# clementabary/music2dance

Hardware: AMD Instinct MI355X
Metric: 120-frame seq/sec, phase3 WGAN-GP step, batch 64 per GPU (higher is better)
Workload: dtype f32

## Files before the change

### music2dance_amd/csrc/gemm_engine.hip

```cpp
#include "gemm_engine.h"
#include <atomic>
#include <map>
#include <mutex>

typedef float f32x16 __attribute__((ext_vector_type(16)));

template <int BM, int BN, int NW>
struct M2dTiling {
  static constexpr int WM = BM >= 64 ? 2 : 1;
  static constexpr int WN = NW / WM;
  static constexpr int TM = BM / (32 * WM);
  static constexpr int TN = BN / (32 * WN);
  static constexpr int NTH = 64 * NW;
};

__device__ __forceinline__ void m2d_divmod(int n, int d, float inv, int& q, int& r) {
  q = (int)((float)n * inv);
  r = n - q * d;
  const int adj = (r < 0 ? -1 : 0) + (r >= d ? 1 : 0);
  q += adj;
  r -= adj * d;
}

__device__ __forceinline__ void m2d_tile_of(int tile_map, int& bx, int& by) {
  bx = blockIdx.x;
  by = blockIdx.y;
  if (tile_map == 0) return;
  const int nt = gridDim.x, mt = gridDim.y;
  const int T = nt * mt, q = T >> 3, r = T & 7;
  const int lin = by * nt + bx;
  const int xcd = lin & 7, idx = lin >> 3;
  const int id = (xcd < r ? xcd * (q + 1) : r * (q + 1) + (xcd - r) * q) + idx;
  const int GM = 8;
  const int per = GM * nt;
  const int grp = id / per, rem = id - grp * per;
  const int first = grp * GM;
  const int gsz = mt - first < GM ? mt - first : GM;
  const int nn = rem / gsz;
  by = first + rem - nn * gsz;
  bx = nn;
}

#define M2D_OOB 0x80000000u
#define M2D_BAD 0x40000000

__device__ __forceinline__ __amdgpu_buffer_rsrc_t m2d_rsrc(const float* p, unsigned nbytes) {
  return __builtin_amdgcn_make_buffer_rsrc((void*)p, (short)0, (int)nbytes, 0x00020000);
}

__device__ __forceinline__ float m2d_bload(__amdgpu_buffer_rsrc_t r, unsigned voff, int soff) {
  return __builtin_bit_cast(float, __builtin_amdgcn_raw_buffer_load_b32(r, (int)voff, soff, 0));
}

typedef __attribute__((address_space(3))) float m2d_lds_f;
__device__ __forceinline__ void m2d_bload_lds(__amdgpu_buffer_rsrc_t r, float* dst, unsigned voff, int soff) {
  __builtin_amdgcn_raw_ptr_buffer_load_lds(r, (m2d_lds_f*)dst, 4, (int)voff, soff, 0, 0);
}

__device__ __forceinline__ int m2d_hi_offset(const M2dOperand& op, int hi) {
  if (op.rdiv2 <= 0) return hi * op.r_hi_stride;
  int q, r;
  m2d_divmod(hi, op.rdiv2, op.rdiv2_inv, q, r);
  return q * op.r_hi2_stride + r * op.r_hi_stride;
}

template <bool KF, int BR, bool MASKED, int NTH = 256>
struct TileMap {
  static constexpr int NE = BR * M2D_BK / NTH;
  static constexpr int NR = KF ? NE : 1;
  static constexpr int NM = MASKED ? NE : 1;
  unsigned eoff[NR];
  int posr;
  int kb;
  unsigned lim_eff;
  bool force_one;
  float one_val;
  float v[NE];
  float mv[NM];

  __device__ __forceinline__ void prep(const M2dOperand& op, int row0, int tid) {
    lim_eff = op.lim > 0 ? (unsigned)op.lim : (unsigned)(M2D_BAD - 1);
    force_one = false;
    one_val = 1.f;
    if constexpr (KF) {
      kb = tid % M2D_BK;
      posr = 0;
#pragma unroll
      for (int i = 0; i < NE; ++i) {
        const int g = row0 + tid / M2D_BK + i * (NTH / M2D_BK);
        const bool rv = g < op.nrows;
        int hi, lo;
        m2d_divmod(rv ? g : 0, op.rdiv, op.rdiv_inv, hi, lo);
        const int off = m2d_hi_offset(op, hi) + lo * op.r_lo_stride + op.r_off + kb * op.k_lo_stride;
        eoff[i] = rv ? ((unsigned)off << 2) : M2D_OOB;
      }
    } else {
      const int kb_t = (tid / BR) * NE;
      kb = BR >= 64 ? __builtin_amdgcn_readfirstlane(kb_t) : kb_t;
      const int g = row0 + tid % BR;
      const bool rv = g < op.nrows;
      force_one = (g + 1 == op.ones_row_p1);
      int hi, lo;
      m2d_divmod(rv ? g : 0, op.rdiv, op.rdiv_inv, hi, lo);
      const int off = m2d_hi_offset(op, hi) + lo * op.r_lo_stride + op.r_off + kb * op.k_lo_stride;
      eoff[0] = (unsigned)off << 2;
      posr = rv ? (op.lim > 0 ? lo * op.r_pos_mul + op.r_pos_off + kb * op.k_pos_lo : 0) : M2D_BAD;
    }
  }

  static constexpr int DL_KSTEP = BR >= 64 ? 1 : 64 / BR;
  __device__ __forceinline__ void prep_dl(const M2dOperand& op, int row0, int tid) {
    static_assert(!KF && !MASKED && (BR == 32 || BR >= 64), "LDS-direct staging: row-fast, unmasked");
    static_assert(BR >= 64 || NTH == 256, "32-row LDS-direct staging: four waves");
    if constexpr (BR >= 64) {
      prep(op, row0, tid);
    } else {
      lim_eff = op.lim > 0 ? (unsigned)op.lim : (unsigned)(M2D_BAD - 1);
      force_one = false;
      kb = 4 * (tid >> 6) + ((tid >> 5) & 1);
      const int g = row0 + (tid & (BR - 1));
      const bool rv = g < op.nrows;
      int hi, lo;
      m2d_divmod(rv ? g : 0, op.rdiv, op.rdiv_inv, hi, lo);
      const int off = m2d_hi_offset(op, hi) + lo * op.r_lo_stride + op.r_off + kb * op.k_lo_stride;
      eoff[0] = (unsigned)off << 2;
      posr = rv ? (op.lim > 0 ? lo * op.r_pos_mul + op.r_pos_off + kb * op.k_pos_lo : 0) : M2D_BAD;
    }
  }

  __device__ __forceinline__ void fetch(__amdgpu_buffer_rsrc_t rs, __amdgpu_buffer_rsrc_t rm, int i, unsigned voff,
                                        int soff) {
    v[i] = m2d_bload(rs, voff, soff);
    if constexpr (MASKED) mv[i] = m2d_bload(rm, voff, soff);
  }

  template <bool UNIFORM>
  __device__ __forceinline__ void load(const M2dOperand& op, __amdgpu_buffer_rsrc_t rs, __amdgpu_buffer_rsrc_t rm,
                                       int hi, int lo0, int kdiv) {
    int hoff = hi * op.k_hi_stride;
    if (op.kdiv2 > 0) {
      const int q = hi / op.kdiv2;
      hoff = q * op.k_hi2_stride + (hi - q * op.kdiv2) * op.k_hi_stride;
    }
    const int S = (hoff + lo0 * op.k_lo_stride) << 2;
    if constexpr (!KF) one_val = hi >= op.ones_from_hi ? 1.f : 0.f;
    if constexpr (KF) {
      if constexpr (UNIFORM) {
#pragma unroll
        for (int i = 0; i < NE; ++i) fetch(rs, rm, i, eoff[i], S);
      } else {
        const bool tv = lo0 + kb < kdiv;
#pragma unroll
        for (int i = 0; i < NE; ++i) fetch(rs, rm, i, tv ? eoff[i] : M2D_OOB, S);
      }
    } else {
      const int P = hi * op.k_pos_hi + lo0 * op.k_pos_lo;
      const unsigned full = eoff[0] + (unsigned)S;
      const int ls4 = op.k_lo_stride << 2;
      if constexpr (UNIFORM) {
        const unsigned voff = ((unsigned)(posr + P) < lim_eff) ? full : M2D_OOB;
#pragma unroll
        for (int i = 0; i < NE; ++i) fetch(rs, rm, i, voff, i * ls4);
      } else {
#pragma unroll
        for (int i = 0; i < NE; ++i) {
          const int pp = (lo0 + kb + i < kdiv) ? P + i * op.k_pos_lo : M2D_BAD;
          fetch(rs, rm, i, ((unsigned)(posr + pp) < lim_eff) ? full + (unsigned)(i * ls4) : M2D_OOB, 0);
        }
      }
    }
  }

  template <bool UNIFORM, int LD>
  __device__ __forceinline__ void load_lds(const M2dOperand& op, __amdgpu_buffer_rsrc_t rs, int hi, int lo0, int kdiv,
                                           float* img, int tid) const {
    static_assert(!KF && !MASKED, "LDS-direct staging: row-fast, unmasked");
    constexpr int KS = DL_KSTEP;
    int hoff = hi * op.k_hi_stride;
    const int S = (hoff + lo0 * op.k_lo_stride) << 2;
    const int P = hi * op.k_pos_hi + lo0 * op.k_pos_lo;
    const unsigned full = eoff[0] + (unsigned)S;
    const int ls4 = (op.k_lo_stride * KS) << 2;
    const int kb0 = BR >= 64 ? kb : 4 * (__builtin_amdgcn_readfirstlane(tid) >> 6);
    const int row0 = BR >= 64 ? (__builtin_amdgcn_readfirstlane(tid) & (BR - 1) & ~63) : 0;
    float* dst = img + kb0 * LD + row0;
    if constexpr (UNIFORM) {
      const unsigned voff = ((unsigned)(posr + P) < lim_eff) ? full : M2D_OOB;
#pragma unroll
      for (int i = 0; i < NE; ++i) m2d_bload_lds(rs, dst + (KS * i) * LD, voff, i * ls4);
    } else {
#pragma unroll
      for (int i = 0; i < NE; ++i) {
        const int pp = (lo0 + kb + KS * i < kdiv) ? P + (KS * i) * op.k_pos_lo : M2D_BAD;
        m2d_bload_lds(rs, dst + (KS * i) * LD, ((unsigned)(posr + pp) < lim_eff) ? full + (unsigned)(i * ls4) : M2D_OOB, 0);
      }
    }
  }

  template <int LD>
  __device__ __forceinline__ void store(const M2dOperand& op, float* s, int tid) const {
#pragma unroll
    for (int i = 0; i < NE; ++i) {
      const int kl = KF ? (tid % M2D_BK) : ((tid / BR) * NE + i);
      const int rl = KF ? (tid / M2D_BK + i * (NTH / M2D_BK)) : (tid % BR);
      float x = v[i];
      if constexpr (MASKED) x *= (mv[i] > 0.f ? 1.f : op.mask_slope);
      if constexpr (!KF) x = force_one ? one_val : x;
      s[kl * LD + rl] = x;
    }
  }
};

struct ChunkCursor {
  int hi, lo0, kdiv, nhi;
  int lo_outer;
  int a_lo, a_hi, b_lo, b_hi;
  __device__ __forceinline__ void seek(int c, int cph) {
    if (lo_outer) {
      const int blk = c / nhi;
      hi = c - blk * nhi;
      lo0 = blk * M2D_BK;
    } else {
      hi = c / cph;
      lo0 = (c - hi * cph) * M2D_BK;
    }
  }
  __device__ __forceinline__ bool past() const { return lo_outer ? lo0 >= kdiv : hi >= nhi; }
  __device__ __forceinline__ bool uniform() const {
    return (!past()) & (lo0 + M2D_BK <= kdiv) & (lo0 >= a_lo) & (lo0 + M2D_BK <= a_hi) & (lo0 >= b_lo) &
           (lo0 + M2D_BK <= b_hi);
  }
  __device__ __forceinline__ int extent() const { return past() ? 0 : kdiv; }
  __device__ __forceinline__ void next() {
    if (lo_outer) {
      hi += 1;
      const bool wrap = hi >= nhi;
      hi = wrap ? 0 : hi;
      lo0 += wrap ? M2D_BK : 0;
    } else {
      lo0 += M2D_BK;
      const bool wrap = lo0 >= kdiv;
      lo0 = wrap ? 0 : lo0;
      hi += wrap ? 1 : 0;
    }
  }
};

__device__ __forceinline__ unsigned m2d_mask_off(unsigned voff, unsigned wrapb) {
  return (voff != M2D_OOB && voff >= wrapb) ? voff - wrapb : voff;
}

__device__ __forceinline__ float m2d_epilogue(const M2dOutMap& o, float v, int row, int col, int addr) {
  const int maddr = (o.mask_wrap && addr >= (int)o.mask_wrap) ? addr - (int)o.mask_wrap : addr;
  if (o.bias_mode == 1) v += o.bias[row];
  else if (o.bias_mode == 2) v += o.bias[col];
  v = m2d_act(v, o.act, o.slope);
  if (o.mask_last) {
    if (o.residual) v += o.residual[addr];
    if (o.mask) v *= (o.mask[maddr] > 0.f ? 1.f : o.mask_slope);
    return v;
  }
  if (o.mask) v *= (o.mask[maddr] > 0.f ? 1.f : o.mask_slope);
  if (o.sum_out) {
    o.sum_out[addr] = v + o.residual[addr];
    return v;
  }
  if (o.residual) v += o.residual[addr];
  return v;
}

template <int BM, int BN, bool AKF, bool BKF, bool MASKED>
__device__ __forceinline__ void m2d_chunk_mma(const TileMap<AKF, BM, MASKED>& ta, const TileMap<BKF, BN, MASKED>& tb,
                                              const M2dOperand& A, const M2dOperand& B, float* smem, int cur,
                                              int tid, int wm, int wn, int l31, int lh,
                                              f32x16 (&acc)[BM / (32 * (BM >= 64 ? 2 : 1))][BN / (32 * (4 / (BM >= 64 ? 2 : 1)))]) {
  constexpr int LDA = BM + M2D_LDPAD;
  constexpr int LDB = BN + M2D_LDPAD;
  constexpr int WM = BM >= 64 ? 2 : 1;
  constexpr int WN = 4 / WM;
  constexpr int TM = BM / (32 * WM);
  constexpr int TN = BN / (32 * WN);
  constexpr int STAGE = M2D_BK * (LDA + LDB);
  const float* as = smem + cur * STAGE + wm * (TM * 32) + l31;
  const float* bs = smem + cur * STAGE + M2D_BK * LDA + wn * (TN * 32) + l31;
  float fa[M2D_BK / 2][TM], fb[M2D_BK / 2][TN];
#pragma unroll
  for (int kk = 0; kk < M2D_BK / 2; ++kk) {
#pragma unroll
    for (int i = 0; i < TM; ++i) fa[kk][i] = as[(2 * kk + lh) * LDA + i * 32];
#pragma unroll
    for (int j = 0; j < TN; ++j) fb[kk][j] = bs[(2 * kk + lh) * LDB + j * 32];
  }
#pragma unroll
  for (int kk = 0; kk < M2D_BK / 2; ++kk)
#pragma unroll
    for (int i = 0; i < TM; ++i)
#pragma unroll
      for (int j = 0; j < TN; ++j)
        acc[i][j] = __builtin_amdgcn_mfma_f32_32x32x2f32(fa[kk][i], fb[kk][j], acc[i][j], 0, 0, 0);
  float* nxt = smem + (cur ^ 1) * STAGE;
  ta.template store<LDA>(A, nxt, tid);
  tb.template store<LDB>(B, nxt + M2D_BK * LDA, tid);
  __builtin_amdgcn_sched_group_barrier(0x100, 4, 0);
#pragma unroll
  for (int kk = 0; kk < M2D_BK / 2; ++kk) {
    __builtin_amdgcn_sched_group_barrier(0x008, TM * TN, 0);
    if (kk < M2D_BK / 2 - 2) __builtin_amdgcn_sched_group_barrier(0x100, 2, 0);
  }
}

template <int BM, int BN, int NW = 4>
__device__ __forceinline__ void m2d_acc_init(const M2dGemmParams& p, const M2dOutMap& O, int N, int split, int m0, int n0, int wm,
                                             int wn, int l31, int lh,
                                             f32x16 (&acc)[M2dTiling<BM, BN, NW>::TM][M2dTiling<BM, BN, NW>::TN]) {
  constexpr int TM = M2dTiling<BM, BN, NW>::TM;
  constexpr int TN = M2dTiling<BM, BN, NW>::TN;
  const bool with_bias = O.bias_mode != 0 && (p.splits <= 1 || (p.tickets && split == 0));
  if (!with_bias) {
#pragma unroll
    for (int i = 0; i < TM; ++i)
#pragma unroll
      for (int j = 0; j < TN; ++j)
#pragma unroll
        for (int r = 0; r < 16; ++r) acc[i][j][r] = 0.f;
    return;
  }
  if (O.bias_mode == 1) {
#pragma unroll
    for (int i = 0; i < TM; ++i)
#pragma unroll
      for (int r = 0; r < 16; ++r) {
        const int row = m0 + wm * (TM * 32) + i * 32 + (r & 3) + 8 * (r >> 2) + 4 * lh;
        const float b = row < p.M ? O.bias[row] : 0.f;
#pragma unroll
        for (int j = 0; j < TN; ++j) acc[i][j][r] = b;
      }
  } else {
#pragma unroll
    for (int j = 0; j < TN; ++j) {
      const int col = n0 + wn * (TN * 32) + j * 32 + l31;
      const float b = col < N ? O.bias[col] : 0.f;
#pragma unroll
      for (int i = 0; i < TM; ++i)
#pragma unroll
        for (int r = 0; r < 16; ++r) acc[i][j][r] = b;
    }
  }
}

__device__ __forceinline__ float4 m2d_ld4(const float* p) { return *reinterpret_cast<const float4*>(p); }
__device__ __forceinline__ void m2d_st4(float* p, float4 v) { *reinterpret_cast<float4*>(p) = v; }

typedef unsigned int m2d_u32x4 __attribute__((__vector_size__(16)));
typedef float m2d_vf32x4 __attribute__((__vector_size__(16)));
__device__ __forceinline__ void m2d_bstore1(__amdgpu_buffer_rsrc_t r, unsigned voff, float v) {
  __builtin_amdgcn_raw_buffer_store_b32(__builtin_bit_cast(unsigned, v), r, (int)voff, 0, 0);
}
__device__ __forceinline__ void m2d_bstore4(__amdgpu_buffer_rsrc_t r, unsigned voff, float4 v) {
  m2d_vf32x4 w;
  w[0] = v.x; w[1] = v.y; w[2] = v.z; w[3] = v.w;
  __builtin_amdgcn_raw_buffer_store_b128(__builtin_bit_cast(m2d_u32x4, w), r, (int)voff, 0, 0);
}
__device__ __forceinline__ float4 m2d_bload4(__amdgpu_buffer_rsrc_t r, unsigned voff) {
  const m2d_vf32x4 w = __builtin_bit_cast(m2d_vf32x4, __builtin_amdgcn_raw_buffer_load_b128(r, (int)voff, 0, 0));
  return make_float4(w[0], w[1], w[2], w[3]);
}

template <int BM, int BN, bool WIDE, int NW = 4>
__device__ __forceinline__ void m2d_tile_epilogue(const M2dGemmParams& p, const M2dOutMap& O, int N, int split, int m0,
                                                  int n0, int wm, int wn, int lane, float* wl,
                                                  f32x16 (&acc)[M2dTiling<BM, BN, NW>::TM][M2dTiling<BM, BN, NW>::TN]) {
  constexpr int WN = M2dTiling<BM, BN, NW>::WN;
  constexpr int TM = M2dTiling<BM, BN, NW>::TM;
  constexpr int TN = M2dTiling<BM, BN, NW>::TN;
  const int l31 = lane & 31, lh = lane >> 5;
  const bool slab = p.splits > 1 && !p.tickets;
  const bool stats = O.row_part != nullptr && !slab;
  const bool has_mask = O.mask != nullptr && !slab, has_res = O.residual != nullptr && !slab;
  const bool two_out = O.sum_out != nullptr && !slab;
  const int act = slab ? 0 : O.act;
  const float ms = O.mask_slope;
  const int m_stride = slab ? p.N : O.m_stride;
  const int m_div = slab ? 0 : O.m_div;
  const int c_lim = slab ? 0 : O.c_lim;
  const int redirect = slab ? 0 : O.redirect_col_p1;
  const float* out_base = slab ? p.slab + (size_t)split * p.M * p.N : O.out;
#define M2D_RS(ptr) m2d_rsrc((ptr), 0x7ffffffcu)
  constexpr int NT = (BM == 128 && WIDE) ? TN : 1;
  const int rl0 = lane >> 3, c4 = (lane & 7) * 4;
  constexpr int PER_TILE = WIDE ? 4 : 16;
  constexpr int ITEMS = NT * PER_TILE;
  constexpr int GROUP = WIDE ? ITEMS : (BM == 128 ? 8 : 16);
#pragma unroll
  for (int i = 0; i < TM; ++i) {
    const int rowb = m0 + wm * (TM * 32) + i * 32;
#pragma unroll
    for (int j0 = 0; j0 < TN; j0 += NT) {
#pragma unroll
      for (int jj = 0; jj < NT; ++jj)
#pragma unroll
        for (int r = 0; r < 16; ++r) wl[jj * 1024 + ((r & 3) + 8 * (r >> 2) + 4 * lh) * 32 + l31] = acc[i][j0 + jj][r];
      __builtin_amdgcn_fence(__ATOMIC_RELEASE, "wavefront");
      __builtin_amdgcn_wave_barrier();
      __builtin_amdgcn_sched_barrier(0);
      int caddr_t[NT], pos_t[NT];
      bool cok_t[NT], red_t[NT];
#pragma unroll
      for (int jj = 0; jj < NT; ++jj) {
        const int col = n0 + wn * (TN * 32) + (j0 + jj) * 32 + (WIDE ? c4 : l31);
        const bool cv = col < N;
        if (slab) {
          caddr_t[jj] = col;
          pos_t[jj] = 0;
        } else {
          int chi, clo;
          m2d_divmod(cv ? col : 0, O.cdiv, O.cdiv_inv, chi, clo);
          caddr_t[jj] = chi * O.c_hi_stride + clo * (WIDE ? 1 : O.c_lo_stride) + O.c_off;
          pos_t[jj] = clo * O.c_pos_mul + O.c_pos_off;
        }
        red_t[jj] = !WIDE && cv && (col + 1 == redirect);
        bool cok = cv;
        if (!WIDE && c_lim > 0 && m_div <= 0) cok = cok && ((unsigned)pos_t[jj] < (unsigned)c_lim);
        cok_t[jj] = cok;
      }
      {
        bool fast = !has_res && m_div <= 0;
        if constexpr (!WIDE) fast = fast && (!stats || (!has_mask && c_lim <= 0 && (p.stats_narrow_fast != 0))) && __ballot(red_t[0]) == 0ull;
        if (fast) {
          if constexpr (!WIDE) {
            if (stats) {
#pragma unroll
              for (int jj = 0; jj < NT; ++jj) {
                const int colb = n0 + wn * (TN * 32) + (j0 + jj) * 32 + c4;
#pragma unroll
                for (int it = 0; it < 4; ++it) {
                  const int rl = rl0 + 8 * it;
                  float4 x = m2d_ld4(wl + jj * 1024 + rl * 32 + c4);
                  x.x = colb + 0 < N ? m2d_act_sel(x.x, act, O.slope) : 0.f;
                  x.y = colb + 1 < N ? m2d_act_sel(x.y, act, O.slope) : 0.f;
                  x.z = colb + 2 < N ? m2d_act_sel(x.z, act, O.slope) : 0.f;
                  x.w = colb + 3 < N ? m2d_act_sel(x.w, act, O.slope) : 0.f;
                  float a1 = (x.x + x.y) + (x.z + x.w);
                  float a2 = (x.x * x.x + x.y * x.y) + (x.z * x.z + x.w * x.w);
#pragma unroll
                  for (int off = 4; off > 0; off >>= 1) {
                    a1 += __shfl_xor(a1, off, 64);
                    a2 += __shfl_xor(a2, off, 64);
                  }
                  if ((lane & 7) == 0 && rowb + rl < p.M) {
                    float* dst = O.row_part + ((size_t)(((n0 / BN) * WN + wn) * TN + j0 + jj) * p.M + rowb + rl) * 2;
                    dst[0] = a1;
                    dst[1] = a2;
                  }
                }
              }
            }
          }
          const __amdgpu_buffer_rsrc_t rso = m2d_rsrc(out_base, 0x7ffffffcu);
#pragma unroll
          for (int jj = 0; jj < NT; ++jj) {
            constexpr int NI = PER_TILE;
            constexpr int RS = WIDE ? 8 : 2;
            const int r0 = WIDE ? rl0 : lh;
            const unsigned step = (unsigned)(RS * m_stride) << 2;
            const unsigned v0 = cok_t[jj] ? (unsigned)((rowb + r0) * m_stride + caddr_t[jj]) << 2 : M2D_OOB;
            const int nrow = p.M - rowb - r0;
            unsigned keep = 0xffffffffu;
            if (has_mask) {
              const __amdgpu_buffer_rsrc_t rsm = m2d_rsrc(O.mask, 0x7ffffffcu);
              const unsigned wrapb = O.mask_wrap ? O.mask_wrap * 4u : 0xffffffffu;
              keep = 0u;
              if constexpr (WIDE) {
                float4 mraw[NI];
#pragma unroll
                for (int it = 0; it < NI; ++it)
                  mraw[it] = m2d_bload4(rsm, m2d_mask_off((RS * it < nrow && v0 != M2D_OOB) ? v0 + (unsigned)it * step : M2D_OOB, wrapb));
#pragma unroll
                for (int it = 0; it < NI; ++it)
                  keep |= ((mraw[it].x > 0.f ? 1u : 0u) | (mraw[it].y > 0.f ? 2u : 0u) | (mraw[it].z > 0.f ? 4u : 0u) | (mraw[it].w > 0.f ? 8u : 0u)) << (4 * it);
              } else {
                float mraw[NI];
#pragma unroll
                for (int it = 0; it < NI; ++it)
                  mraw[it] = m2d_bload(rsm, m2d_mask_off((RS * it < nrow && v0 != M2D_OOB) ? v0 + (unsigned)it * step : M2D_OOB, wrapb), 0);
#pragma unroll
                for (int it = 0; it < NI; ++it) keep |= (mraw[it] > 0.f ? 1u : 0u) << it;
              }
            }
            const float* img = wl + jj * 1024 + r0 * 32 + (WIDE ? c4 : l31);
#pragma unroll
            for (int it = 0; it < NI; ++it) {
              const bool ok = RS * it < nrow && v0 != M2D_OOB;
              const unsigned voff = ok ? v0 + (unsigned)it * step : M2D_OOB;
              if constexpr (WIDE) {
                float4 x = m2d_ld4(img + it * (RS * 32));
                const unsigned kb = keep >> (4 * it);
                x.x = m2d_act(x.x, act, O.slope) * ((kb & 1u) ? 1.f : ms);
                x.y = m2d_act(x.y, act, O.slope) * ((kb & 2u) ? 1.f : ms);
                x.z = m2d_act(x.z, act, O.slope) * ((kb & 4u) ? 1.f : ms);
                x.w = m2d_act(x.w, act, O.slope) * ((kb & 8u) ? 1.f : ms);
                m2d_bstore4(rso, voff, x);
                if (stats) {
                  float a1 = ok ? (x.x + x.y) + (x.z + x.w) : 0.f;
                  float a2 = ok ? (x.x * x.x + x.y * x.y) + (x.z * x.z + x.w * x.w) : 0.f;
#pragma unroll
                  for (int off = 4; off > 0; off >>= 1) {
                    a1 += __shfl_xor(a1, off, 64);
                    a2 += __shfl_xor(a2, off, 64);
                  }
                  if ((lane & 7) == 0 && RS * it < nrow) {
                    float* dst = O.row_part + ((size_t)(((n0 / BN) * WN + wn) * TN + j0 + jj) * p.M + rowb + r0 + RS * it) * 2;
                    dst[0] = a1;
                    dst[1] = a2;
                  }
                }
              } else {
                float x = img[it * (RS * 32)];
                x = m2d_act_sel(x, act, O.slope) * (((keep >> it) & 1u) ? 1.f : ms);
                m2d_bstore1(rso, voff, x);
              }
            }
          }
          __builtin_amdgcn_wave_barrier();
          continue;
        }
      }
      auto locate = [&](int q, int& jj, int& rl, int& row, unsigned& voff) {
        jj = NT > 1 ? q / PER_TILE : 0;
        const int it = q - jj * PER_TILE;
        rl = WIDE ? rl0 + 8 * it : 2 * it + lh;
        row = rowb + rl;
        const int caddr = NT > 1 && jj ? caddr_t[NT - 1] : caddr_t[0];
        bool ok = row < p.M && (NT > 1 && jj ? cok_t[NT - 1] : cok_t[0]) && !(NT > 1 && jj ? red_t[NT - 1] : red_t[0]);
        int addr;
        if (!WIDE && m_div > 0) {
          int mhi, mlo;
          m2d_divmod(row, m_div, 1.f / (float)m_div, mhi, mlo);
          const int pos = NT > 1 && jj ? pos_t[NT - 1] : pos_t[0];
          if (c_lim > 0) ok = ok && ((unsigned)(pos + mlo * O.m_pos_mul) < (unsigned)c_lim);
          addr = mhi * m_stride + mlo * O.m_lo_stride + caddr;
        } else {
          addr = row * m_stride + caddr;
        }
        voff = ok ? (unsigned)addr << 2 : M2D_OOB;
      };
#pragma unroll 1
      for (int q0 = 0; q0 < ITEMS; q0 += GROUP) {
        unsigned keep = 0xffffffffu;
        if (has_mask) {
          keep = 0u;
          const unsigned wrapb = O.mask_wrap ? O.mask_wrap * 4u : 0xffffffffu;
          if constexpr (WIDE) {
            float4 mraw[GROUP];
#pragma unroll
            for (int q = 0; q < GROUP; ++q) {
              int jj, rl, row;
              unsigned voff;
              locate(q0 + q, jj, rl, row, voff);
              mraw[q] = m2d_bload4(M2D_RS(O.mask), m2d_mask_off(voff, wrapb));
            }
#pragma unroll
            for (int q = 0; q < GROUP; ++q)
              keep |= ((mraw[q].x > 0.f ? 1u : 0u) | (mraw[q].y > 0.f ? 2u : 0u) | (mraw[q].z > 0.f ? 4u : 0u) | (mraw[q].w > 0.f ? 8u : 0u)) << (4 * q);
          } else {
            float mraw[GROUP];
#pragma unroll
            for (int q = 0; q < GROUP; ++q) {
              int jj, rl, row;
              unsigned voff;
              locate(q0 + q, jj, rl, row, voff);
              mraw[q] = m2d_bload(M2D_RS(O.mask), m2d_mask_off(voff, wrapb), 0);
            }
#pragma unroll
            for (int q = 0; q < GROUP; ++q) keep |= (mraw[q] > 0.f ? 1u : 0u) << q;
          }
        }
#pragma unroll 2
        for (int qq = 0; qq < GROUP; ++qq) {
          int jj, rl, row;
          unsigned voff;
          locate(q0 + qq, jj, rl, row, voff);
          const bool ok = voff != M2D_OOB;
          float a1 = 0.f, a2 = 0.f;
          if constexpr (WIDE) {
            float4 x = m2d_ld4(wl + jj * 1024 + rl * 32 + c4);
            x.x = m2d_act(x.x, act, O.slope); x.y = m2d_act(x.y, act, O.slope);
            x.z = m2d_act(x.z, act, O.slope); x.w = m2d_act(x.w, act, O.slope);
            if (has_res && O.mask_last) {
              const float4 r4 = m2d_bload4(M2D_RS(O.residual), voff);
              x.x += r4.x; x.y += r4.y; x.z += r4.z; x.w += r4.w;
            }
            const unsigned kb = keep >> (4 * qq);
            x.x *= (kb & 1u) ? 1.f : ms; x.y *= (kb & 2u) ? 1.f : ms; x.z *= (kb & 4u) ? 1.f : ms; x.w *= (kb & 8u) ? 1.f : ms;
            if (has_res && !O.mask_last) {
              const float4 r4 = m2d_bload4(M2D_RS(O.residual), voff);
              const float4 sum = make_float4(x.x + r4.x, x.y + r4.y, x.z + r4.z, x.w + r4.w);
              if (two_out) m2d_bstore4(M2D_RS(O.sum_out), voff, sum);
              else x = sum;
            }
            m2d_bstore4(M2D_RS(out_base), voff, x);
            if (stats) {
              a1 = ok ? (x.x + x.y) + (x.z + x.w) : 0.f;
              a2 = ok ? (x.x * x.x + x.y * x.y) + (x.z * x.z + x.w * x.w) : 0.f;
#pragma unroll
              for (int off = 4; off > 0; off >>= 1) {
                a1 += __shfl_xor(a1, off, 64);
                a2 += __shfl_xor(a2, off, 64);
              }
              if ((lane & 7) == 0 && row < p.M) {
                float* dst = O.row_part + ((size_t)(((n0 / BN) * WN + wn) * TN + j0 + jj) * p.M + row) * 2;
                dst[0] = a1;
                dst[1] = a2;
              }
            }
// ... 373 lines not shown
    const int nq = top >= 0 ? (top / s - qmin + 1) : 0;
    if (nq <= 0) return;
    N = p.ph_batch * nq;
    if ((int)(bx * BN) >= N) return;
    nhi = taps;
    A.r_off += r * (p.ph_a_step ? p.ph_a_step : p.ph_cout);
    B.nrows = N;
    B.rdiv = nq;
    B.rdiv_inv = 1.f / (float)nq;
    B.r_off = qmin;
    B.r_pos_off = qmin;
    O.cdiv = nq;
    O.cdiv_inv = B.rdiv_inv;
    O.c_off = s * qmin + r - p.ph_pad;
    O.c_pos_off = O.c_off;
  }
  const int m0 = by * BM;
  const int n0 = bx * BN;
  TileMap<false, BM, false, NTH> ta;
  TileMap<false, BN, false, NTH> tb;
  ta.prep_dl(A, m0, tid);
  tb.prep_dl(B, n0, tid);
  const __amdgpu_buffer_rsrc_t ra = m2d_rsrc(A.base, A.nbytes);
  const __amdgpu_buffer_rsrc_t rb = m2d_rsrc(B.base, B.nbytes);

  f32x16 acc[TM][TN];
  if constexpr (EPI == 2) {
#pragma unroll
    for (int i = 0; i < TM; ++i)
#pragma unroll
      for (int j = 0; j < TN; ++j)
#pragma unroll
        for (int r = 0; r < 16; ++r) acc[i][j][r] = 0.f;
  } else {
    m2d_acc_init<BM, BN, NW>(p, O, N, split, m0, n0, wm, wn, l31, lh, acc);
  }

  const int cph = (p.kdiv + M2D_BK - 1) / M2D_BK;
  const int nchunks = nhi * cph;
  const int cps = (nchunks + p.splits - 1) / p.splits;
  const int c0 = split * cps;
  const int c1 = (c0 + cps < nchunks) ? (c0 + cps) : nchunks;

  if (c0 < c1) {
    ChunkCursor cc;
    cc.kdiv = p.kdiv;
    cc.nhi = nhi;
    cc.lo_outer = p.lo_outer;
    cc.seek(c0, cph);
    cc.a_lo = A.k_safe_lo; cc.a_hi = A.k_safe_hi;
    cc.b_lo = B.k_safe_lo; cc.b_hi = B.k_safe_hi;
    ta.template load_lds<false, BM>(A, ra, cc.hi, cc.lo0, cc.extent(), smem, tid);
    tb.template load_lds<false, BN>(B, rb, cc.hi, cc.lo0, cc.extent(), smem + M2D_BK * BM, tid);
    cc.next();
    asm volatile("s_waitcnt vmcnt(0)" ::: "memory");
    __syncthreads();
    M2D_STAMP_AT(1);
    for (int c = c0; c < c1; ++c) {
      const int cur = (c - c0) & 1;
      float* nxt = smem + (cur ^ 1) * STAGE;
      if (cc.uniform()) {
        ta.template load_lds<true, BM>(A, ra, cc.hi, cc.lo0, cc.kdiv, nxt, tid);
        tb.template load_lds<true, BN>(B, rb, cc.hi, cc.lo0, cc.kdiv, nxt + M2D_BK * BM, tid);
      } else {
        ta.template load_lds<false, BM>(A, ra, cc.hi, cc.lo0, cc.extent(), nxt, tid);
        tb.template load_lds<false, BN>(B, rb, cc.hi, cc.lo0, cc.extent(), nxt + M2D_BK * BM, tid);
      }
      m2d_chunk_mma_dl<BM, BN, NW>(smem + cur * STAGE, wm, wn, l31, lh, acc);
      cc.next();
      asm volatile("s_waitcnt vmcnt(0)" ::: "memory");
      __syncthreads();
    }
  }
  M2D_STAMP_AT(2);
  if (p.tickets && !m2d_splitk_fixup<BM, BN, NW>(p, split, tid, reinterpret_cast<volatile int*>(smem), acc)) return;
  if constexpr (EPI == 2) m2d_tile_epilogue_quad<BM, BN, NW>(p, O, N, m0, n0, wm, wn, l31, lh, acc);
  else m2d_tile_epilogue<BM, BN, EPI == 1, NW>(p, O, N, split, m0, n0, wm, wn, lane, smem + wave * ((BM == 128 && NW == 4) ? 2048 : 1024), acc);
#ifdef M2D_STAMP
  asm volatile("s_waitcnt vmcnt(0)" ::: "memory");
#endif
  M2D_STAMP_AT(3);
}

template <int RB>
__device__ __forceinline__ void m2d_chunk_mma_tall(const float* stage, int wn, int l31, int lh, f32x16 (&acc)[4]) {
  const float* as = stage + l31;
  const float* bs = stage + M2D_BK * 128 + wn * 32 + l31;
  float fa[M2D_BK / 2][RB], fb[M2D_BK / 2];
#pragma unroll
  for (int kk = 0; kk < M2D_BK / 2; ++kk) {
#pragma unroll
    for (int i = 0; i < RB; ++i) fa[kk][i] = as[(2 * kk + lh) * 128 + i * 32];
    fb[kk] = bs[(2 * kk + lh) * 128];
  }
#pragma unroll
  for (int kk = 0; kk < M2D_BK / 2; ++kk)
#pragma unroll
    for (int i = 0; i < RB; ++i) acc[i] = __builtin_amdgcn_mfma_f32_32x32x2f32(fa[kk][i], fb[kk], acc[i], 0, 0, 0);
  __builtin_amdgcn_sched_group_barrier(0x100, RB + 1, 0);
#pragma unroll
  for (int kk = 0; kk < M2D_BK / 2; ++kk) {
    __builtin_amdgcn_sched_group_barrier(0x008, RB, 0);
    if (kk < M2D_BK / 2 - 2) __builtin_amdgcn_sched_group_barrier(0x100, RB > 1 ? 3 : 2, 0);
  }
}

__global__ void __launch_bounds__(256, 2) m2d_gemm_dl_tall_kernel(const M2dGemmParams p) {
  constexpr int BM = 128, BN = 128;
  constexpr int STAGE = M2D_BK * (BM + BN);
  __shared__ float smem[2 * STAGE];
  const int tid = threadIdx.x;
  const int lane = tid & 63;
  const int wn = tid >> 6;
  const int l31 = lane & 31;
  const int lh = lane >> 5;
  M2D_STAMP_AT(0);
  const M2dOperand& A = p.A;
  const M2dOperand& B = p.B;
  const M2dOutMap& O = p.O;
  const int N = p.N;
  int bx, by;
  m2d_tile_of(p.tile_map, bx, by);
  const int m0 = by * BM;
  const int n0 = bx * BN;
  TileMap<false, BM, false, 256> ta;
  TileMap<false, BN, false, 256> tb;
  ta.prep_dl(A, m0, tid);
  tb.prep_dl(B, n0, tid);
  const __amdgpu_buffer_rsrc_t ra = m2d_rsrc(A.base, A.nbytes);
  const __amdgpu_buffer_rsrc_t rb = m2d_rsrc(B.base, B.nbytes);
  f32x16 acc[4];
#pragma unroll
  for (int i = 0; i < 4; ++i)
#pragma unroll
    for (int r = 0; r < 16; ++r) acc[i][r] = 0.f;

  const int nhi = p.nhi;
  const int cph = (p.kdiv + M2D_BK - 1) / M2D_BK;
  ChunkCursor cc;
  cc.kdiv = p.kdiv;
  cc.nhi = nhi;
  cc.lo_outer = 1;
  cc.seek(0, cph);
  cc.a_lo = A.k_safe_lo; cc.a_hi = A.k_safe_hi;
  cc.b_lo = B.k_safe_lo; cc.b_hi = B.k_safe_hi;
  ta.template load_lds<false, BM>(A, ra, cc.hi, cc.lo0, cc.extent(), smem, tid);
  tb.template load_lds<false, BN>(B, rb, cc.hi, cc.lo0, cc.extent(), smem + M2D_BK * BM, tid);
  cc.next();
  asm volatile("s_waitcnt vmcnt(0)" ::: "memory");
  __syncthreads();
  M2D_STAMP_AT(1);
  int cur = 0;
  auto stage_next = [&]() {
    float* nxt = smem + (cur ^ 1) * STAGE;
    if (cc.uniform()) {
      ta.template load_lds<true, BM>(A, ra, cc.hi, cc.lo0, cc.kdiv, nxt, tid);
      tb.template load_lds<true, BN>(B, rb, cc.hi, cc.lo0, cc.kdiv, nxt + M2D_BK * BM, tid);
    } else {
      ta.template load_lds<false, BM>(A, ra, cc.hi, cc.lo0, cc.extent(), nxt, tid);
      tb.template load_lds<false, BN>(B, rb, cc.hi, cc.lo0, cc.extent(), nxt + M2D_BK * BM, tid);
    }
  };
  auto step_done = [&]() {
    cc.next();
    asm volatile("s_waitcnt vmcnt(0)" ::: "memory");
    __syncthreads();
// ... 462 lines not shown
      const double lat = (double)m2d_ceil_div64(per_cu, conc) * step;
      double cost = 8.0 + cps * (thr > lat ? thr : lat);
      if (sp > 1) cost += 6.0 + slab_mul * (double)sp * (double)M * (double)N * 8.0 / 4.0e6;
      if (rm) cost = rounds_cost(*rm, b, tiles * sp, cps, sp, M, N);
      if (rm && kind == M2D_PLAN_BWD_WEIGHT && bms[b] < 128 && M >= 128) cost *= 2.0;
      all[na].bm = bms[b];
      all[na].splits = (int)sp;
      all[na].cost = cost;
      ++na;
    }
  }
  for (int i = 0; i < na; ++i)
    for (int j = i + 1; j < na; ++j)
      if (all[j].cost < all[i].cost) {
        PlanCand t = all[i];
        all[i] = all[j];
        all[j] = t;
      }
  int n = 0;
  for (int i = 0; i < na && n < M2D_MAX_CAND; ++i)
    if (all[i].cost <= 1.5 * all[0].cost + 6.0) out[n++] = all[i];
  return n;
}

#ifdef M2D_TUNING
static int g_last_plan[9];
extern "C" int m2d_debug_last_plan(int* out) {
  memcpy(out, g_last_plan, sizeof(g_last_plan));
  return M2D_OK;
}
#endif

M2dGemmPlan m2d_gemm_plan(int M, int N, int nchunks, int phases, bool allow_split, double small_tile_penalty, int kind) {
  PlanCand c[M2D_MAX_CAND];
  const int n = plan_candidates(M, N, nchunks, phases, allow_split, small_tile_penalty, c, kind);
  M2dGemmPlan pl;
  pl.bm = n ? c[0].bm : 128;
  pl.splits = n ? c[0].splits : 1;
  pl.ws_bytes = 0;
  for (int i = 0; i < n; ++i) {
    const size_t b = m2d_slab_bytes(M, N, c[i].bm, c[i].splits);
    if (b > pl.ws_bytes) pl.ws_bytes = b;
  }
#ifdef M2D_TUNING
  if (const char* e = getenv("M2D_PLAN")) {
    int bm = 0, sp = 0;
    if (sscanf(e, "%d,%d", &bm, &sp) == 2) {
      if (bm == 32 || bm == 64 || bm == 128) pl.bm = bm;
      if (sp >= 1 && allow_split && phases <= 1 && sp <= nchunks) pl.splits = sp;
      if (sp == 1) pl.splits = 1;
      const size_t b = m2d_slab_bytes(M, N, pl.bm, pl.splits);
      if (b > pl.ws_bytes) pl.ws_bytes = b;
    }
  }
#endif
  return pl;
}

template <int BM, bool AKF, bool BKF>
static void launch_tile(const M2dGemmParams& p, dim3 grid, hipStream_t stream) {
  const bool masked = p.A.mask || p.B.mask;
  if (masked && p.O.wide) hipLaunchKernelGGL((m2d_gemm_kernel<BM, 128, AKF, BKF, true, true>), grid, dim3(256), 0, stream, p);
  else if (masked) hipLaunchKernelGGL((m2d_gemm_kernel<BM, 128, AKF, BKF, true, false>), grid, dim3(256), 0, stream, p);
  else if (p.O.wide) hipLaunchKernelGGL((m2d_gemm_kernel<BM, 128, AKF, BKF, false, true>), grid, dim3(256), 0, stream, p);
  else hipLaunchKernelGGL((m2d_gemm_kernel<BM, 128, AKF, BKF, false, false>), grid, dim3(256), 0, stream, p);
}

static bool dl_enabled() {
  static const bool on = [] { const char* e = getenv("M2D_DL"); return !(e && e[0] == '0'); }();
  return on;
}
bool m2d_dl_enabled() { return dl_enabled(); }

static inline bool dl_eligible(const M2dGemmParams& p, bool akf, bool bkf) {
  return !akf && !bkf && !p.A.mask && !p.B.mask && !p.A.ones_row_p1 && !p.B.ones_row_p1 && p.A.rdiv2 <= 0 &&
         p.B.rdiv2 <= 0 && p.A.kdiv2 <= 0 && p.B.kdiv2 <= 0;
}

static bool dl8_enabled() {
  static const bool on = [] { const char* e = getenv("M2D_DL8"); return !(e && e[0] == '0'); }();
  return on;
}

template <int BM>
static int launch_maps(const M2dGemmParams& p, bool akf, bool bkf, dim3 grid, hipStream_t stream) {
  {
    if (dl_enabled() && dl_eligible(p, akf, bkf)) {
      if constexpr (BM == 128) {
        if (p.tall_last_rb) {
          hipLaunchKernelGGL(m2d_gemm_dl_tall_kernel, grid, dim3(256), 0, stream, p);
          return 0;
        }
        if (dl8_enabled() && (p.O.wide || (p.O.quad && p.splits <= 1))) {
          if (p.O.wide) hipLaunchKernelGGL((m2d_gemm_dl_kernel<128, 128, 1, 8>), grid, dim3(512), 0, stream, p);
          else hipLaunchKernelGGL((m2d_gemm_dl_kernel<128, 128, 2, 8>), grid, dim3(512), 0, stream, p);
          return 0;
        }
      }
      if (p.O.wide) hipLaunchKernelGGL((m2d_gemm_dl_kernel<BM, 128, 1>), grid, dim3(256), 0, stream, p);
      else if (p.O.quad && p.splits <= 1) hipLaunchKernelGGL((m2d_gemm_dl_kernel<BM, 128, 2>), grid, dim3(256), 0, stream, p);
      else hipLaunchKernelGGL((m2d_gemm_dl_kernel<BM, 128, 0>), grid, dim3(256), 0, stream, p);
      return 0;
    }
  }
  if (akf && !bkf) launch_tile<BM, true, false>(p, grid, stream);
  else if (!akf && !bkf) launch_tile<BM, false, false>(p, grid, stream);
  else if (akf && bkf) launch_tile<BM, true, true>(p, grid, stream);
  else return -1;
  return 0;
}

static std::mutex g_scratch_mu;
static std::map<hipStream_t, std::pair<unsigned*, size_t>> g_scratch;

unsigned* m2d_stream_scratch_get(hipStream_t stream, size_t* bytes) {
  std::lock_guard<std::mutex> lk(g_scratch_mu);
  auto it = g_scratch.find(stream);
  if (it == g_scratch.end()) {
    if (bytes) *bytes = 0;
    return nullptr;
  }
  if (bytes) *bytes = it->second.second;
  return it->second.first;
}

extern "C" int m2d_stream_create(void** stream) {
  if (!stream) M2D_FAIL(M2D_ERR_ARG, "m2d_stream_create: null argument");
  hipStream_t s = nullptr;
  if (hipStreamCreateWithFlags(&s, hipStreamNonBlocking) != hipSuccess) M2D_FAIL(M2D_ERR_HIP, "m2d_stream_create: hipStreamCreateWithFlags failed");
  *stream = (void*)s;
  return M2D_OK;
}

extern "C" int m2d_stream_scratch_set(void* stream, void* zeroed, size_t bytes) {
  std::lock_guard<std::mutex> lk(g_scratch_mu);
  if (!zeroed || bytes == 0) g_scratch.erase((hipStream_t)stream);
  else g_scratch[(hipStream_t)stream] = std::make_pair((unsigned*)zeroed, bytes);
  return M2D_OK;
}

struct PlanQuery {
  int nchunks, phases;
  bool allow_split;
  double small_tile_penalty;
  int kind;
  bool k4;
  void* ws;
  size_t ws_bytes;
  unsigned* tickets;
  size_t ticket_bytes;
  const char* what;
};
struct Plan {
  int bm, splits;
  unsigned* tickets;
};

static unsigned* decide_fused(const M2dGemmParams& p, const PlanQuery& q, int bm, int splits) {
  static const bool on = [] { const char* e = getenv("M2D_FUSED_SPLITK"); return !(e && e[0] == '0'); }();
  static const int max_splits = [] { const char* e = getenv("M2D_FUSE_MAX"); return e ? atoi(e) : M2D_FUSE_MAX_SPLITS; }();
  if (!on || splits <= 1 || splits > max_splits || p.bwd_data || !q.ws) return nullptr;
  const size_t need = m2d_slab_bytes(p.M, p.N, bm, splits);
  if (need > q.ws_bytes || need >= 0x7fffffffULL || ((uintptr_t)q.ws & 15u)) return nullptr;
  const size_t tiles = (size_t)m2d_ceil_div(p.M, bm) * (size_t)m2d_ceil_div(p.N, 128);
  if (!q.tickets || tiles * sizeof(unsigned) > q.ticket_bytes) return nullptr;
  return q.tickets;
}

static bool stats_split_enabled() {
  static const bool on = [] { const char* e = getenv("M2D_STATS_SPLIT"); return !(e && e[0] == '0'); }();
  return on;
}

static int select_plan(const M2dGemmParams& p, const PlanQuery& q, Plan* out) {
  const bool stats = p.O.row_part != nullptr;
  const bool allow_split = q.allow_split && !(stats && !stats_split_enabled());
// ... 189 lines not shown
```

Measured before the change: 5702.

## Add paired-row LDS-direct GEMM kernel with 16-byte A staging and interleaved rows

Adds a new 128x128 four-wave GEMM kernel for eligible problems. It stages A with 16-byte buffer-to-LDS loads and interleaves row pairs so each lane reads a float2 fragment feeding two MFMA tiles. The B loader, bias init and epilogue are adapted to the paired row mapping. The goal is fewer LDS-direct load instructions and fewer LDS reads per chunk than the 8-wave and 4-wave DL kernels, in exchange for stricter alignment and eligibility checks. It is enabled by default through an environment mask and also counts its launches.

```diff
diff --git a/music2dance_amd/csrc/gemm_engine.hip b/music2dance_amd/csrc/gemm_engine.hip
--- a/music2dance_amd/csrc/gemm_engine.hip
+++ b/music2dance_amd/csrc/gemm_engine.hip
@@ -78,6 +78,7 @@
   float v[NE];
   float mv[NM];
 
+  template <bool PAIRS = false>
   __device__ __forceinline__ void prep(const M2dOperand& op, int row0, int tid) {
     lim_eff = op.lim > 0 ? (unsigned)op.lim : (unsigned)(M2D_BAD - 1);
     force_one = false;
@@ -97,7 +98,9 @@
     } else {
       const int kb_t = (tid / BR) * NE;
       kb = BR >= 64 ? __builtin_amdgcn_readfirstlane(kb_t) : kb_t;
-      const int g = row0 + tid % BR;
+      int rl = tid % BR;
+      if constexpr (PAIRS) rl = (rl & ~63) + 32 * (tid & 1) + ((tid & 63) >> 1);
+      const int g = row0 + rl;
       const bool rv = g < op.nrows;
       force_one = (g + 1 == op.ones_row_p1);
       int hi, lo;
@@ -109,11 +112,13 @@
   }
 
   static constexpr int DL_KSTEP = BR >= 64 ? 1 : 64 / BR;
+  template <bool PAIRS = false>
   __device__ __forceinline__ void prep_dl(const M2dOperand& op, int row0, int tid) {
     static_assert(!KF && !MASKED && (BR == 32 || BR >= 64), "LDS-direct staging: row-fast, unmasked");
     static_assert(BR >= 64 || NTH == 256, "32-row LDS-direct staging: four waves");
+    static_assert(!PAIRS || BR >= 64, "paired rows: whole 64-row lines");
     if constexpr (BR >= 64) {
-      prep(op, row0, tid);
+      prep<PAIRS>(op, row0, tid);
     } else {
       lim_eff = op.lim > 0 ? (unsigned)op.lim : (unsigned)(M2D_BAD - 1);
       force_one = false;
@@ -198,6 +203,32 @@
   }
 
   template <int LD>
+  __device__ __forceinline__ void load_lds_merged(const M2dOperand& op, __amdgpu_buffer_rsrc_t rs, int hi, int lo0, int kdiv,
+                                                  bool uniform, float* img, int tid) const {
+    static_assert(!KF && !MASKED && BR >= 64, "LDS-direct staging: row-fast, unmasked, whole 64-row lines");
+    const int S = (hi * op.k_hi_stride + lo0 * op.k_lo_stride) << 2;
+    const int P = hi * op.k_pos_hi + lo0 * op.k_pos_lo;
+    const unsigned full = eoff[0] + (unsigned)S;
+    const int ls4 = op.k_lo_stride << 2;
+    float* dst = img + kb * LD + (__builtin_amdgcn_readfirstlane(tid) & (BR - 1) & ~63);
+    unsigned voff[NE];
+    if (uniform) {
+      const unsigned v = ((unsigned)(posr + P) < lim_eff) ? full : M2D_OOB;
+#pragma unroll
+      for (int i = 0; i < NE; ++i) voff[i] = v;
+    } else {
+#pragma unroll
+      for (int i = 0; i < NE; ++i) {
+        const int pp = (lo0 + kb + i < kdiv) ? P + i * op.k_pos_lo : M2D_BAD;
+        voff[i] = ((unsigned)(posr + pp) < lim_eff) ? full + (unsigned)(i * ls4) : M2D_OOB;
+      }
+    }
+    const int lsu = uniform ? ls4 : 0;
+#pragma unroll
+    for (int i = 0; i < NE; ++i) m2d_bload_lds(rs, dst + i * LD, voff[i], i * lsu);
+  }
+
+  template <int LD>
   __device__ __forceinline__ void store(const M2dOperand& op, float* s, int tid) const {
 #pragma unroll
     for (int i = 0; i < NE; ++i) {
@@ -309,7 +340,14 @@
   }
 }
 
-template <int BM, int BN, int NW = 4>
+template <bool PAIR>
+struct M2dAccRows {
+  static constexpr int STEP = PAIR ? 2 : 1;
+  static __device__ __forceinline__ int first(int w0, int i) { return PAIR ? w0 + i : w0 + 32 * i; }
+  static __device__ __forceinline__ int row(int w0, int i, int f) { return first(w0, i) + STEP * f; }
+};
+
+template <int BM, int BN, int NW = 4, bool PAIR = false>
 __device__ __forceinline__ void m2d_acc_init(const M2dGemmParams& p, const M2dOutMap& O, int N, int split, int m0, int n0, int wm,
                                              int wn, int l31, int lh,
                                              f32x16 (&acc)[M2dTiling<BM, BN, NW>::TM][M2dTiling<BM, BN, NW>::TN]) {
@@ -330,7 +368,7 @@
     for (int i = 0; i < TM; ++i)
 #pragma unroll
       for (int r = 0; r < 16; ++r) {
-        const int row = m0 + wm * (TM * 32) + i * 32 + (r & 3) + 8 * (r >> 2) + 4 * lh;
+        const int row = M2dAccRows<PAIR>::row(m0 + wm * (TM * 32), i, (r & 3) + 8 * (r >> 2) + 4 * lh);
         const float b = row < p.M ? O.bias[row] : 0.f;
 #pragma unroll
         for (int j = 0; j < TN; ++j) acc[i][j][r] = b;
@@ -366,7 +404,7 @@
   return make_float4(w[0], w[1], w[2], w[3]);
 }
 
-template <int BM, int BN, bool WIDE, int NW = 4>
+template <int BM, int BN, bool WIDE, int NW = 4, bool PAIR = false>
 __device__ __forceinline__ void m2d_tile_epilogue(const M2dGemmParams& p, const M2dOutMap& O, int N, int split, int m0,
                                                   int n0, int wm, int wn, int lane, float* wl,
                                                   f32x16 (&acc)[M2dTiling<BM, BN, NW>::TM][M2dTiling<BM, BN, NW>::TN]) {
@@ -393,7 +431,8 @@
   constexpr int GROUP = WIDE ? ITEMS : (BM == 128 ? 8 : 16);
 #pragma unroll
   for (int i = 0; i < TM; ++i) {
-    const int rowb = m0 + wm * (TM * 32) + i * 32;
+    constexpr int RM = M2dAccRows<PAIR>::STEP;
+    const int rowb = M2dAccRows<PAIR>::first(m0 + wm * (TM * 32), i);
 #pragma unroll
     for (int j0 = 0; j0 < TN; j0 += NT) {
 #pragma unroll
@@ -447,8 +486,8 @@
                     a1 += __shfl_xor(a1, off, 64);
                     a2 += __shfl_xor(a2, off, 64);
                   }
-                  if ((lane & 7) == 0 && rowb + rl < p.M) {
-                    float* dst = O.row_part + ((size_t)(((n0 / BN) * WN + wn) * TN + j0 + jj) * p.M + rowb + rl) * 2;
+                  if ((lane & 7) == 0 && rowb + RM * rl < p.M) {
+                    float* dst = O.row_part + ((size_t)(((n0 / BN) * WN + wn) * TN + j0 + jj) * p.M + rowb + RM * rl) * 2;
                     dst[0] = a1;
                     dst[1] = a2;
                   }
@@ -460,11 +499,12 @@
 #pragma unroll
           for (int jj = 0; jj < NT; ++jj) {
             constexpr int NI = PER_TILE;
-            constexpr int RS = WIDE ? 8 : 2;
+            constexpr int IS = WIDE ? 8 : 2;
+            constexpr int RS = RM * IS;
             const int r0 = WIDE ? rl0 : lh;
             const unsigned step = (unsigned)(RS * m_stride) << 2;
-            const unsigned v0 = cok_t[jj] ? (unsigned)((rowb + r0) * m_stride + caddr_t[jj]) << 2 : M2D_OOB;
-            const int nrow = p.M - rowb - r0;
+            const unsigned v0 = cok_t[jj] ? (unsigned)((rowb + RM * r0) * m_stride + caddr_t[jj]) << 2 : M2D_OOB;
+            const int nrow = p.M - rowb - RM * r0;
             unsigned keep = 0xffffffffu;
             if (has_mask) {
               const __amdgpu_buffer_rsrc_t rsm = m2d_rsrc(O.mask, 0x7ffffffcu);
@@ -493,7 +533,7 @@
               const bool ok = RS * it < nrow && v0 != M2D_OOB;
               const unsigned voff = ok ? v0 + (unsigned)it * step : M2D_OOB;
               if constexpr (WIDE) {
-                float4 x = m2d_ld4(img + it * (RS * 32));
+                float4 x = m2d_ld4(img + it * (IS * 32));
                 const unsigned kb = keep >> (4 * it);
                 x.x = m2d_act(x.x, act, O.slope) * ((kb & 1u) ? 1.f : ms);
                 x.y = m2d_act(x.y, act, O.slope) * ((kb & 2u) ? 1.f : ms);
@@ -509,13 +549,13 @@
                     a2 += __shfl_xor(a2, off, 64);
                   }
                   if ((lane & 7) == 0 && RS * it < nrow) {
-                    float* dst = O.row_part + ((size_t)(((n0 / BN) * WN + wn) * TN + j0 + jj) * p.M + rowb + r0 + RS * it) * 2;
+                    float* dst = O.row_part + ((size_t)(((n0 / BN) * WN + wn) * TN + j0 + jj) * p.M + rowb + RM * r0 + RS * it) * 2;
                     dst[0] = a1;
                     dst[1] = a2;
                   }
                 }
               } else {
-                float x = img[it * (RS * 32)];
+                float x = img[it * (IS * 32)];
                 x = m2d_act_sel(x, act, O.slope) * (((keep >> it) & 1u) ? 1.f : ms);
                 m2d_bstore1(rso, voff, x);
               }
@@ -529,7 +569,7 @@
         jj = NT > 1 ? q / PER_TILE : 0;
         const int it = q - jj * PER_TILE;
         rl = WIDE ? rl0 + 8 * it : 2 * it + lh;
-        row = rowb + rl;
+        row = rowb + RM * rl;
         const int caddr = NT > 1 && jj ? caddr_t[NT - 1] : caddr_t[0];
         bool ok = row < p.M && (NT > 1 && jj ? cok_t[NT - 1] : cok_t[0]) && !(NT > 1 && jj ? red_t[NT - 1] : red_t[0]);
         int addr;
@@ -1069,6 +1109,141 @@
   M2D_STAMP_AT(3);
 }
 
+typedef float m2d_f32x2 __attribute__((ext_vector_type(2)));
+
+__device__ __forceinline__ void m2d_chunk_mma_dlp(const float* stage, int wm, int wn, int l31, int lh, f32x16 (&acc)[2][2]) {
+  const float* as = stage + wm * 64 + 2 * l31;
+  const float* bs = stage + M2D_BK * 128 + wn * 64 + 2 * l31;
+  m2d_f32x2 fa[M2D_BK / 2], fb[M2D_BK / 2];
+#pragma unroll
+  for (int kk = 0; kk < M2D_BK / 2; ++kk) {
+    fa[kk] = *reinterpret_cast<const m2d_f32x2*>(as + (2 * kk + lh) * 128);
+    fb[kk] = *reinterpret_cast<const m2d_f32x2*>(bs + (2 * kk + lh) * 128);
+  }
+#pragma unroll
+  for (int kk = 0; kk < M2D_BK / 2; ++kk)
+#pragma unroll
+    for (int i = 0; i < 2; ++i)
+#pragma unroll
+      for (int j = 0; j < 2; ++j)
+        acc[i][j] = __builtin_amdgcn_mfma_f32_32x32x2f32(fa[kk][i], fb[kk][j], acc[i][j], 0, 0, 0);
+  __builtin_amdgcn_sched_group_barrier(0x100, 4, 0);
+#pragma unroll
+  for (int kk = 0; kk < M2D_BK / 2; ++kk) {
+    __builtin_amdgcn_sched_group_barrier(0x008, 4, 0);
+    if (kk < M2D_BK / 2 - 2) __builtin_amdgcn_sched_group_barrier(0x100, 2, 0);
+  }
+}
+
+template <int EPI>
+__global__ void __launch_bounds__(256, 2) m2d_gemm_dlp_kernel(const M2dGemmParams p) {
+  constexpr int BM = 128, BN = 128;
+  static_assert(M2D_BK == 16, "two 128-row lines per 16-byte DMA piece, eight pieces per chunk");
+  constexpr int STAGE = M2D_BK * (BM + BN);
+  __shared__ __attribute__((aligned(16))) float smem[2 * STAGE];
+  const int tid = threadIdx.x;
+  const int lane = tid & 63;
+  const int wave = __builtin_amdgcn_readfirstlane(tid >> 6);
+  const int wm = wave & 1;
+  const int wn = wave >> 1;
+  const int l31 = lane & 31;
+  const int lh = lane >> 5;
+  M2D_STAMP_AT(0);
+
+  M2dOperand A = p.A;
+  M2dOperand B = p.B;
+  M2dOutMap O = p.O;
+  int N = p.N;
+  int nhi = p.nhi;
+  int split = blockIdx.z;
+  int bx, by;
+  m2d_tile_of(p.tile_map, bx, by);
+  if (p.bwd_data) {
+    const int r = blockIdx.z;
+    const int s = p.phases;
+    split = 0;
+    const int taps = r < p.ph_ks ? (p.ph_ks - r + s - 1) / s : 0;
+    const int qmin = r >= p.ph_pad ? 0 : (p.ph_pad - r + s - 1) / s;
+    const int top = p.ph_L - 1 + p.ph_pad - r;
+    const int nq = top >= 0 ? (top / s - qmin + 1) : 0;
+    if (nq <= 0) return;
+    N = p.ph_batch * nq;
+    if ((int)(bx * BN) >= N) return;
+    nhi = taps;
+    A.r_off += r * (p.ph_a_step ? p.ph_a_step : p.ph_cout);
+    B.nrows = N;
+    B.rdiv = nq;
+    B.rdiv_inv = 1.f / (float)nq;
+    B.r_off = qmin;
+    B.r_pos_off = qmin;
+    O.cdiv = nq;
+    O.cdiv_inv = B.rdiv_inv;
+    O.c_off = s * qmin + r - p.ph_pad;
+    O.c_pos_off = O.c_off;
+  }
+  const int m0 = by * BM;
+  const int n0 = bx * BN;
+  unsigned ea[2];
+  int ka[2];
+#pragma unroll
+  for (int i = 0; i < 2; ++i) {
+    ka[i] = 2 * (wave + 4 * i) + lh;
+    ea[i] = (unsigned)(A.r_off + m0 + 4 * l31 + ka[i] * A.k_lo_stride) << 2;
+  }
+  TileMap<false, BN, false, 256> tb;
+  tb.template prep_dl<true>(B, n0, tid);
+  const __amdgpu_buffer_rsrc_t ra = m2d_rsrc(A.base, A.nbytes);
+  const __amdgpu_buffer_rsrc_t rb = m2d_rsrc(B.base, B.nbytes);
+
+  f32x16 acc[2][2];
+  m2d_acc_init<BM, BN, 4, true>(p, O, N, split, m0, n0, wm, wn, l31, lh, acc);
+
+  const int cph = (p.kdiv + M2D_BK - 1) / M2D_BK;
+  const int nchunks = nhi * cph;
+  const int cps = (nchunks + p.splits - 1) / p.splits;
+  const int c0 = split * cps;
+  const int c1 = (c0 + cps < nchunks) ? (c0 + cps) : nchunks;
+
+  if (c0 < c1) {
+    ChunkCursor cc;
+    cc.kdiv = p.kdiv;
+    cc.nhi = nhi;
+    cc.lo_outer = p.lo_outer;
+    cc.seek(c0, cph);
+    cc.a_lo = A.k_safe_lo; cc.a_hi = A.k_safe_hi;
+    cc.b_lo = B.k_safe_lo; cc.b_hi = B.k_safe_hi;
+    auto stage = [&](float* st) {
+      const int ext = cc.extent();
+      const unsigned sa = (unsigned)((cc.hi * A.k_hi_stride + cc.lo0 * A.k_lo_stride) << 2);
+#pragma unroll
+      for (int i = 0; i < 2; ++i)
+        __builtin_amdgcn_raw_ptr_buffer_load_lds(ra, (m2d_lds_f*)(st + (wave + 4 * i) * 256), 16,
+                                                 (int)(cc.lo0 + ka[i] < ext ? ea[i] + sa : M2D_OOB), 0, 0, 0);
+      tb.template load_lds_merged<BN>(B, rb, cc.hi, cc.lo0, ext, cc.uniform(), st + M2D_BK * BM, tid);
+    };
+    stage(smem);
+    cc.next();
+    asm volatile("s_waitcnt vmcnt(0)" ::: "memory");
+    __syncthreads();
+    M2D_STAMP_AT(1);
+    for (int c = c0; c < c1; ++c) {
+      const int cur = (c - c0) & 1;
+      stage(smem + (cur ^ 1) * STAGE);
+      m2d_chunk_mma_dlp(smem + cur * STAGE, wm, wn, l31, lh, acc);
+      cc.next();
+      asm volatile("s_waitcnt vmcnt(0)" ::: "memory");
+      __syncthreads();
+    }
+  }
+  M2D_STAMP_AT(2);
+  if (p.tickets && !m2d_splitk_fixup<BM, BN, 4>(p, split, tid, reinterpret_cast<volatile int*>(smem), acc)) return;
+  m2d_tile_epilogue<BM, BN, EPI == 1, 4, true>(p, O, N, split, m0, n0, wm, wn, lane, smem + wave * 2048, acc);
+#ifdef M2D_STAMP
+  asm volatile("s_waitcnt vmcnt(0)" ::: "memory");
+#endif
+  M2D_STAMP_AT(3);
+}
+
 template <int RB>
 __device__ __forceinline__ void m2d_chunk_mma_tall(const float* stage, int wn, int l31, int lh, f32x16 (&acc)[4]) {
   const float* as = stage + l31;
@@ -1697,6 +1872,20 @@
   return on;
 }
 
+#define M2D_DLP_DEFAULT 3
+static std::atomic<int> g_dlp{[] { const char* e = getenv("M2D_DLP"); return e ? atoi(e) & 3 : M2D_DLP_DEFAULT; }()};
+extern "C" int m2d_debug_dlp_set(int mask) { return g_dlp.exchange(mask < 0 ? M2D_DLP_DEFAULT : mask & 3, std::memory_order_relaxed); }
+static std::atomic<unsigned long long> g_dlp_launches{0};
+extern "C" unsigned long long m2d_debug_dlp_launches(void) { return g_dlp_launches.load(std::memory_order_relaxed); }
+
+static inline bool dlp_eligible(const M2dGemmParams& p) {
+  const M2dOperand& a = p.A;
+  const int phase_step = p.bwd_data ? (p.ph_a_step ? p.ph_a_step : p.ph_cout) : 0;
+  return M2D_BK == 16 && p.M % 128 == 0 && a.nrows >= p.M && a.rdiv == 1 && a.r_hi_stride == 1 && a.lim <= 0 &&
+         ((uintptr_t)a.base & 15u) == 0 && a.r_off % 4 == 0 && a.k_lo_stride % 4 == 0 && a.k_hi_stride % 4 == 0 &&
+         phase_step % 4 == 0 && p.O.m_div <= 0;
+}
+
 template <int BM>
 static int launch_maps(const M2dGemmParams& p, bool akf, bool bkf, dim3 grid, hipStream_t stream) {
   {
@@ -1706,7 +1895,14 @@
           hipLaunchKernelGGL(m2d_gemm_dl_tall_kernel, grid, dim3(256), 0, stream, p);
           return 0;
         }
-        if (dl8_enabled() && (p.O.wide || (p.O.quad && p.splits <= 1))) {
+        const bool eight = dl8_enabled() && (p.O.wide || (p.O.quad && p.splits <= 1));
+        if ((g_dlp.load(std::memory_order_relaxed) & (eight ? 2 : 1)) && dlp_eligible(p) && !(eight && p.splits > 1)) {
+          g_dlp_launches.fetch_add(1, std::memory_order_relaxed);
+          if (p.O.wide) hipLaunchKernelGGL(m2d_gemm_dlp_kernel<1>, grid, dim3(256), 0, stream, p);
+          else hipLaunchKernelGGL(m2d_gemm_dlp_kernel<0>, grid, dim3(256), 0, stream, p);
+          return 0;
+        }
+        if (eight) {
           if (p.O.wide) hipLaunchKernelGGL((m2d_gemm_dl_kernel<128, 128, 1, 8>), grid, dim3(512), 0, stream, p);
           else hipLaunchKernelGGL((m2d_gemm_dl_kernel<128, 128, 2, 8>), grid, dim3(512), 0, stream, p);
           return 0;
```

Result: no change. 5740 (median of 6 runs) (+0.7%).
